# inkandswitch/peritext

Measured on NVIDIA H100. Metric: ops merged/sec across batch, higher is better.
Workload: dtype u32

## Files before the change

### peritext_b200/csrc/engine.cu

```cuda
#include <algorithm>
#include <atomic>
#include <cstdlib>
#include <cstring>
#include <initializer_list>
#include <string>
#include <thread>
#include <utility>
#include <vector>

#include "merge_kernel.cuh"
#include "warp_kernel.cuh"
#include "patch_kernel.cuh"
#include "patch_large_kernel.cuh"
#include "team_kernel.cuh"
#include "render_kernel.cuh"
#include "patch_json_kernel.cuh"
#include "append_kernel.cuh"
#include "change_kernel.cuh"
#include "exchange_kernel.cuh"
#include "changes_json_kernel.cuh"
#include "upload_kernel.cuh"
#include "scan_kernel.cuh"
#include "admit_kernel.cuh"
#include "query_kernel.cuh"
// ... 60 lines not shown

struct pt_batch {
    int device = 0;
    cudaStream_t stream = nullptr;
    int num_sms = 0;
    pt_limits limits{};
    bool have_batch = false, merged = false;
    bool patch_pool_changed = false;
    bool patch_window_changed = false;
    uint32_t n_logs = 0;
    uint64_t n_insdel = 0, n_mark = 0;
    std::vector<pt_log_desc> h_desc;
    ptp::Plan plan;
    DevBuf d_runs, d_tokens, d_run_off, d_tok_off, d_cins, d_cmarks;
    DevBuf d_desc, d_insdel, d_marks, d_order, d_counters, d_results, d_text_off, d_span_off, d_text, d_spans, d_pool, d_slab, d_retry, d_seq;
    DevBuf d_bsum, d_ctoff, d_csoff, d_ctext, d_cspans;
    DevBuf d_cdesc, d_changes, d_deps, d_admit;
    std::vector<pt_change_desc> h_cdesc;
    uint64_t n_changes = 0, n_deps = 0;
    DevBuf d_patch_recs, d_patch_items, d_patch_status;
    DevBuf d_patch_first;
    DevBuf d_large_cand, d_large_scratch;
    HostBuf h_patch_recs, h_patch_items, h_patch_status, h_patch_misc, h_patch_first;
    DevBuf d_jval, d_jvoff, d_jlink, d_jloff, d_jcom, d_jcoff;
    JsonBufs spans_json, patches_json;
    JsonBufs changes_json;
    HostBuf h_cj_status;
    DevBuf d_picnt, d_piseg, d_pibsum, d_pitmp, d_pisorted;
    uint64_t patch_cap = 0;
    bool have_changes = false;
    uint32_t adm_maxR = 1;
    const pt_insdel_rec* dp_insdel = nullptr;
    const pt_mark_rec* dp_marks = nullptr;
    HostBuf h_stage, h_results, h_text, h_spans, h_pool, h_misc, h_seq, h_ctoff, h_csoff;
    HostBuf h_chg_status, h_chg_desc, h_chg_insdel, h_chg_marks;
    HostBuf h_xch_totals, h_xch_status, h_xch_off, h_xch_delivered, h_xch_desc;
    bool have_actors = false;
    DevBuf d_anames, d_aoff, d_afirst;
    std::vector<uint64_t> h_afirst, h_abyte;
    std::vector<char> h_adense;
    HostBuf h_act_data, h_act_off, h_act_first;
    HostBuf h_syn_totals, h_syn_status, h_syn_off, h_syn_aoff, h_syn_amap;
    HostBuf h_add_totals, h_add_rank, h_add_aoff, h_add_amap;
    cudaEvent_t ev0 = nullptr, ev1 = nullptr;
    cudaStream_t side = nullptr, launch_stream = nullptr;
    cudaEvent_t ev_fork = nullptr, ev_join = nullptr;
    uint64_t launches = 0;
    cudaGraphExec_t graph_exec = nullptr;
    bool graph_ok = false, graph_tried = false;
    uint32_t merges_since_upload = 0;
    bool dl_begun = false;
    uint32_t kernels_per_merge = 0;
    uint64_t pool_used_host = 0;
};

namespace {

DevCounters* counters(const pt_batch* b) { return (DevCounters*)b->d_counters.p; }

void drop_graph(pt_batch* b) {
    if (b->graph_exec) cudaGraphExecDestroy(b->graph_exec);
    b->graph_exec = nullptr; b->graph_ok = false; b->graph_tried = false; b->merges_since_upload = 0;
}

cudaError_t launched(pt_batch* b) {
    const cudaError_t e = cudaGetLastError();
// ... 168 lines not shown
        }
    }
    switch (k) {
        case 1: return launch_bin_t<kCtaBins[1].block>(b, k, P, retry);
        case 2: return launch_bin_t<kCtaBins[2].block>(b, k, P, retry);
        case 3: return launch_bin_t<kCtaBins[3].block>(b, k, P, retry);
        default: return launch_bin_t<kCtaBins[4].block>(b, k, P, retry);
    }
}

int install_plan(pt_batch* b, const pt_packed_ops& ops, ptp::Plan&& plan, bool own_records) {
    b->n_logs = ops.n_logs; b->n_insdel = ops.n_insdel_total; b->n_mark = ops.n_mark_total;
    b->h_desc.assign(ops.logs, ops.logs + ops.n_logs);
    b->plan = std::move(plan);
    int rc;
    if ((rc = alloc_and_upload_plan(b))) return rc;
    if (own_records) {
        if ((rc = reserve_n<pt_insdel_rec>(b->d_insdel, b->n_insdel))) return rc;
        if ((rc = reserve_n<pt_mark_rec>(b->d_marks, b->n_mark))) return rc;
    }
    return PT_OK;
}

int begin_upload(pt_batch* b, const pt_packed_ops& ops, bool own_records) {
    PT_CUDA(cudaSetDevice(b->device));
    PT_CUDA(cudaStreamSynchronize(b->stream));
    b->have_batch = false; b->merged = false; b->dl_begun = false; b->have_changes = false; b->have_actors = false;
    drop_graph(b);
    ptp::Plan plan;
    if (const char* err = ptp::make_plan(ops, b->limits, b->num_sms, plan)) { g_last_error = err; return PT_ERR_INVALID; }
    return install_plan(b, ops, std::move(plan), own_records);
}

int finish_upload(pt_batch* b, const void* insdel, const void* marks, std::initializer_list<std::pair<const void*, uint64_t>> sources) {
    bool pageable = false;
    for (const auto& s : sources) {
        if (!s.second) continue;
        cudaPointerAttributes a;
        if (cudaPointerGetAttributes(&a, s.first) != cudaSuccess) { cudaGetLastError(); pageable = true; }
        else if (a.type != cudaMemoryTypeHost) pageable = true;
    }
    if (pageable) PT_CUDA(cudaStreamSynchronize(b->stream));
    b->dp_insdel = (const pt_insdel_rec*)insdel; b->dp_marks = (const pt_mark_rec*)marks;
    b->have_batch = true;
    return PT_OK;
}

template <class Q, class A, class Launch>
int run_queries(pt_batch* b, const char* fn, const char* verb, const Q* queries, uint32_t n, A* out, Launch launch) {
    if (!b || (n && (!queries || !out))) return PT_ERR_INVALID;
    if (!b->merged) { g_last_error = std::string(verb) + " before merge"; return PT_ERR_STATE; }
    if (!(b->limits.flags & PT_FLAG_EMIT_SEQUENCE)) { g_last_error = "the handle was created without PT_FLAG_EMIT_SEQUENCE"; return PT_ERR_STATE; }
    if (!n) return PT_OK;
    PT_CUDA(cudaSetDevice(b->device));
    DevBuf dq, da;
    int rc;
    if ((rc = dq.reserve((size_t)n * sizeof(Q))) || (rc = da.reserve((size_t)n * sizeof(A)))) return rc;
    cudaError_t e = cudaMemcpyAsync(dq.p, queries, (size_t)n * sizeof(Q), cudaMemcpyHostToDevice, b->stream);
    if (e == cudaSuccess) {
        launch(warp_grid(b, n, 128), 128u, (const Q*)dq.p, (A*)da.p);
        e = launched(b);
    }
    if (e == cudaSuccess) e = cudaMemcpyAsync(out, da.p, (size_t)n * sizeof(A), cudaMemcpyDeviceToHost, b->stream);
    if (e == cudaSuccess) e = cudaStreamSynchronize(b->stream);
    if (e != cudaSuccess) { g_last_error = std::string(fn) + ": " + cudaGetErrorString(e); return PT_ERR_CUDA; }
    return PT_OK;
}

int load_json_pools(pt_batch* b, const pt_json_pools* pools, const char* fn, ptr::JsonPools* P) {
    struct Pool { const uint8_t* data; const uint64_t* off; uint64_t count; DevBuf* dd; DevBuf* doff; const char* name; };
    const Pool ps[3] = {{pools->values, pools->values_off, pools->n_values, &b->d_jval, &b->d_jvoff, "values"},
                        {pools->links, pools->links_off, pools->n_links, &b->d_jlink, &b->d_jloff, "links"},
                        {pools->comments, pools->comments_off, pools->n_comments, &b->d_jcom, &b->d_jcoff, "comments"}};
    for (const Pool& p : ps) {
        if (p.count && (!p.data || !p.off)) { g_last_error = std::string(fn) + ": null " + p.name + " pool with a nonzero count"; return PT_ERR_INVALID; }
        for (uint64_t k = 0; k < p.count; k++)
// ... 402 lines not shown
        n_ch = n ? ncd[n - 1].change_off + ncd[n - 1].n_changes : 0; n_dp = n ? ncd[n - 1].dep_off + ncd[n - 1].n_deps : 0;
        if ((rc = upload_n(b, dcdesc, dch->logs, n)) || (rc = upload_n(b, ncdesc, ncd.data(), n)) ||
            (rc = reserve_n<pt_change_rec>(nch, n_ch)) || (rc = reserve_n<pt_dep_rec>(ndp, n_dp))) return rc;
        const pt_change_rec* d_dchg = dch->changes;
        const pt_dep_rec* d_ddep = dch->deps;
        if (!table_on_device) {
            if ((rc = upload_n(b, dchg, dch->changes, dch->n_changes_total)) || (rc = upload_n(b, ddep, dch->deps, dch->n_deps_total))) return rc;
            d_dchg = (const pt_change_rec*)dchg.p; d_ddep = (const pt_dep_rec*)ddep.p;
        }
        if (n) {
            pta::splice_changes_kernel<<<warp_grid(b, n, threads), threads, 0, b->stream>>>(
                (const pt_change_desc*)b->d_cdesc.p, (const pt_change_desc*)ncdesc.p, (const pt_change_desc*)dcdesc.p, n, DR,
                (const pt_change_rec*)b->d_changes.p, (const pt_dep_rec*)b->d_deps.p, d_dchg, d_ddep, (pt_change_rec*)nch.p, (pt_dep_rec*)ndp.p);
            PT_CUDA(launched(b));
        }
    }
    uint32_t bad = 0;
    PT_CUDA(cudaMemcpyAsync(&bad, abad.p, 4, cudaMemcpyDeviceToHost, b->stream));
    PT_CUDA(cudaStreamSynchronize(b->stream));
    if (bad) { g_last_error = std::string(fn) + "a resident comment rank is outside comment_map"; return PT_ERR_INVALID; }
    bool keep_actors = !(R.actor_off && R.actor_off[n] > R.actor_off[0]) && !(R.ctr_off && R.ctr_off[n] > R.ctr_off[0]);
    for (uint32_t i = 0; keep_actors && i < n; i++) keep_actors = nd[i].n_actors == b->h_desc[i].n_actors;
    b->have_actors = b->have_actors && keep_actors;
    b->have_batch = false; b->merged = false; b->dl_begun = false;
    drop_graph(b);
    b->d_insdel.swap(nins); b->d_marks.swap(nmarks);
    if (dch) {
        b->d_cdesc.swap(ncdesc); b->d_changes.swap(nch); b->d_deps.swap(ndp);
        b->h_cdesc = std::move(ncd); b->n_changes = n_ch; b->n_deps = n_dp; b->adm_maxR = maxR;
    }
    if ((rc = install_plan(b, ops, std::move(plan), true))) return rc;
    PT_CUDA(cudaStreamSynchronize(b->stream));
    b->dp_insdel = (const pt_insdel_rec*)b->d_insdel.p; b->dp_marks = (const pt_mark_rec*)b->d_marks.p;
    b->have_batch = true;
    return PT_OK;
}

int pt_batch_append(pt_batch* b, const pt_packed_ops* delta, const pt_append_remap* remap, const pt_change_table* dch) {
    if (!b || !delta || (delta->n_logs && !delta->logs)) return PT_ERR_INVALID;
    if (!b->have_batch) { g_last_error = "pt_batch_append before pt_batch_upload"; return PT_ERR_STATE; }
    return splice_append(b, "pt_batch_append: ", delta, false, remap ? *remap : pt_append_remap{}, dch, false);
}

static std::string check_change(const pt_batch* b, const pt_change_input& in, std::vector<pt_log_desc>& dd, std::vector<uint32_t>& new_elems,
                                std::vector<uint32_t>& work) {
    const uint32_t n = b->n_logs;
    if (in.n_logs != n) return "the input has " + std::to_string(in.n_logs) + " logs and the batch " + std::to_string(n);
    if (!n) return std::string();
    if (!in.actor || !in.input_off) return "null actor or input_off";
    if (in.input_off[0] != 0) return "input_off[0] is not 0";
    if ((in.input_off[n] && !in.ops) || (in.n_tokens && !in.tokens)) return "null ops or tokens with a nonzero count";
    dd.resize(n); new_elems.assign(n, 0);
    uint64_t io = 0, mo = 0;
    for (uint32_t i = 0; i < n; i++) {
        const pt_log_desc& L = b->h_desc[i];
        const uint64_t lo = in.input_off[i], hi = in.input_off[i + 1];
        if (hi < lo) return "input_off decreases at log " + std::to_string(i);
        dd[i] = pt_log_desc{io, mo, 0, 0, L.n_actors, L.max_ctr};
        const uint32_t A = in.actor[i];
        if (A == PT_CHANGE_NO_ACTOR) {
            if (hi > lo) return at(i) + "InputOperations without an actor";
            continue;
        }
        if (A >= L.n_actors) return at(i) + "actor rank " + std::to_string(A) + " >= the log's " + std::to_string(L.n_actors) + " actors";
        uint64_t next = (uint64_t)L.max_ctr + 1, last = L.max_ctr, nid = 0, nmk = 0, nel = 0;
        for (uint64_t k = lo; k < hi; k++) {
// ... 544 lines not shown
    if (count) {
        pty::AddParams A{};
        A.n_logs = n; A.T = pty::Tables{(const uint8_t*)b->d_anames.p, (const unsigned long long*)b->d_aoff.p, (const unsigned long long*)b->d_afirst.p};
        A.data = (const uint8_t*)ddata.p; A.off = (const unsigned long long*)doff.p; A.first = (const unsigned long long*)dfirst.p;
        A.fresh = (uint32_t*)dfresh.p; A.new_id = (unsigned long long*)dnew.p; A.totals = (pty::SyncTotals*)dtot.p;
        pty::add_select_kernel<<<warp_grid(b, n, 128), 128, 0, b->stream>>>(A);
        PT_CUDA(launched(b));
        PT_CUDA(cudaMemcpyAsync(tot, dtot.p, (size_t)n * sizeof(pty::SyncTotals), cudaMemcpyDeviceToHost, b->stream));
        PT_CUDA(cudaStreamSynchronize(b->stream));
        for (uint32_t i = 0; i < n; i++) if (tot[i].n_new) grow[i] = i;
    } else {
        for (uint32_t i = 0; i < n; i++) tot[i] = pty::SyncTotals{};
    }
    if ((rc = grow_tables(b, fn, grow, tot, n, (const uint8_t*)ddata.p, (const unsigned long long*)doff.p, (const unsigned long long*)dfirst.p,
                          (const unsigned long long*)dnew.p, b->h_add_aoff, b->h_add_amap, &spliced))) return rc;
    if (count) {
        const pty::Tables T{(const uint8_t*)b->d_anames.p, (const unsigned long long*)b->d_aoff.p, (const unsigned long long*)b->d_afirst.p};
        pty::add_ranks_kernel<<<warp_grid(b, n, 128), 128, 0, b->stream>>>(n, T, (const uint8_t*)ddata.p, (const unsigned long long*)doff.p,
                                                                           (const unsigned long long*)dfirst.p, (uint16_t*)drank.p);
        PT_CUDA(launched(b));
        PT_CUDA(cudaMemcpyAsync(b->h_add_rank.p, drank.p, count * 2, cudaMemcpyDeviceToHost, b->stream));
        PT_CUDA(cudaStreamSynchronize(b->stream));
    }
    *out = pt_actor_view{n, count, (const uint16_t*)b->h_add_rank.p, (const uint64_t*)b->h_add_aoff.p, (const uint16_t*)b->h_add_amap.p, spliced ? 1u : 0u};
    return PT_OK;
}

static int enqueue_merge(pt_batch* b) {
    DevCounters* c = counters(b);
    PT_CUDA(cudaMemsetAsync(c, 0, sizeof(DevCounters), b->stream));
    ptk::BatchParams P{};
    P.desc = (const pt_log_desc*)b->d_desc.p;
    P.insdel = b->dp_insdel; P.marks = b->dp_marks;
    P.results = (pt_log_result*)b->d_results.p;
    P.text_off = (const uint64_t*)b->d_text_off.p; P.span_off = (const uint64_t*)b->d_span_off.p;
    P.text = (uint32_t*)b->d_text.p; P.spans = (pt_span*)b->d_spans.p;
    P.comment_pool = (uint32_t*)b->d_pool.p; P.comment_used = &c->comment_used; P.comment_cap = b->plan.pool_cap;
    P.slab = (char*)b->d_slab.p;
    P.slab_counter = c->slab; P.slab_slots = b->plan.slab_slots;
    P.seq = (b->limits.flags & PT_FLAG_EMIT_SEQUENCE) ? (uint32_t*)b->d_seq.p : nullptr;
    P.stats = c->stats;
    P.admit = nullptr;
    if (b->have_changes && b->n_logs) {
        const auto [wpb, smem] = actor_shape(b->adm_maxR);
        if (smem > 48 * 1024) PT_CUDA(cudaFuncSetAttribute(ptadm::admit_kernel, cudaFuncAttributeMaxDynamicSharedMemorySize, (int)smem));
        ptadm::admit_kernel<<<warp_grid(b, b->n_logs, wpb * 32), wpb * 32, smem, b->stream>>>(
            (const pt_change_desc*)b->d_cdesc.p, (const pt_change_rec*)b->d_changes.p, (const pt_dep_rec*)b->d_deps.p, (const pt_log_desc*)b->d_desc.p,
            b->n_logs, b->adm_maxR, (uint32_t*)b->d_admit.p, (pt_log_result*)b->d_results.p);
        PT_CUDA(launched(b));
        P.admit = (const uint32_t*)b->d_admit.p;
    }
    { const char* e = getenv("PT_PREFETCH"); P.prefetch_next = e ? (uint32_t)atoi(e) : 0u; }
    { const char* e = getenv("PT_WARP_FLAGS"); P.warp_flags = e ? (uint32_t)atoi(e) : 0x704u; }
    { const char* e = getenv("PT_TMA"); P.use_tma = e ? (uint32_t)atoi(e) : 1u; }
    int rc;
    const uint32_t* bin_first = b->plan.bin_first;
    const bool have0 = bin_first[1] > bin_first[0], haveBlocks = bin_first[kNumBins] > bin_first[1];
    const bool fork = have0 && haveBlocks && b->side != nullptr;
    if (fork) {
        PT_CUDA(cudaEventRecord(b->ev_fork, b->stream));
        PT_CUDA(cudaStreamWaitEvent(b->side, b->ev_fork, 0));
        b->launch_stream = b->side;
        for (int k = 1; k < kNumBins; k++) if ((rc = launch_bin(b, k, P, false))) { b->launch_stream = b->stream; return rc; }
        PT_CUDA(cudaEventRecord(b->ev_join, b->side));
        b->launch_stream = b->stream;
        if ((rc = launch_bin(b, 0, P, false))) return rc;
// ... 578 lines not shown
```

### peritext_b200/csrc/merge_kernel.cuh

```cuda
#pragma once
#include <cuda_runtime.h>
#include <stdint.h>

#include "../../include/peritext_b200.h"
#include "../../include/pt_digest.h"

namespace ptk {

struct BatchParams {
    const pt_log_desc* __restrict__ desc;
    const pt_insdel_rec* __restrict__ insdel;
    const pt_mark_rec* __restrict__ marks;
    const uint32_t* __restrict__ order;
    uint32_t n_work;
    uint32_t* work_counter;
    pt_log_result* results;
    const uint64_t* __restrict__ text_off;
    const uint64_t* __restrict__ span_off;
    uint32_t* text;
    pt_span* spans;
    uint32_t* comment_pool;
    unsigned long long* comment_used;
    unsigned long long comment_cap;
    char* slab;
    unsigned long long slab_bytes;
    uint32_t* slab_counter;
    uint32_t slab_slots;
    uint32_t smem_arena_bytes;
    unsigned long long* stats;
    uint32_t* retry_list;
    uint32_t* retry_count;
    const uint32_t* n_work_dev;
    uint32_t prefetch_next;
    uint32_t warp_flags;
    uint32_t use_tma;
    uint32_t* seq;
    const uint32_t* admit;
};

__device__ __forceinline__ uint4 ld_rec(const pt_insdel_rec* p) { return __ldg(reinterpret_cast<const uint4*>(p)); }
__device__ __forceinline__ void prefetch_l2(const void* p) { asm volatile("prefetch.global.L2 [%0];" ::"l"(p)); }

__device__ __forceinline__ uint32_t smem_u32(const void* p) { return (uint32_t)__cvta_generic_to_shared(p); }
__device__ __forceinline__ void mbar_init(unsigned long long* bar, uint32_t count) {
    asm volatile("mbarrier.init.shared::cta.b64 [%0], %1;" ::"r"(smem_u32(bar)), "r"(count) : "memory");
// ... 965 lines not shown
```

### peritext_b200/csrc/plan.cpp

```cpp
#include "plan.h"

#include <algorithm>
#include <cstdio>
#include <cstdlib>
#include <numeric>

namespace ptp {

RouteConfig RouteConfig::from_env() {
    RouteConfig c;
    if (const char* f = getenv("PT_WARP_FORCE")) c.force = atoi(f) != 0;
    if (const char* t = getenv("PT_TEAM")) c.team_on = atoi(t) != 0;
    if (const char* pw = getenv("PT_PATCH_WARP")) c.patch_warp_on = atoi(pw) != 0;
    if (const char* w = getenv("PT_WARP")) {
        unsigned long a, wp, sl, ct;
        if (sscanf(w, "%lu:%lu:%lu:%lu", &a, &wp, &sl, &ct) == 4) {
            if (sl < 256) sl *= 1024;
            sl &= ~(unsigned long)15;
            if ((wp == 2 || wp == 4 || wp == 8) && sl * wp <= 227 * 1024) c.warp = BinCfg{(uint32_t)a, (int)wp * 32, (uint32_t)sl, (int)ct};
        } else if (atoi(w) == 0) {
            c.warp_on = false; c.team_on = false;
        }
    }
    return c;
}

Route route_of(const pt_log_desc& L, const RouteConfig& cfg, bool emit_sequence) {
    const uint64_t n = L.n_insdel, m = L.n_mark, R = L.n_actors ? L.n_actors : 1, recs = n + m, KS = (uint64_t)L.max_ctr * R;
    const bool key16 = !emit_sequence && KS < 0xFFFFull;
    if (cfg.warp_on && key16 && recs <= cfg.warp.max_recs) {
        const bool packed3 = R == 3 && n <= 1022, compact = R >= 3 && R <= 30 && n <= 2046;
        const uint64_t idbytes = packed3 ? 4ull * L.max_ctr : compact ? 2ull * L.max_ctr + 512 : 2 * KS;
        const uint64_t rest = packed3 ? n / 2 + 32 + 14 * (n / 4) + (KS / 32 + 2) * 6 + 512 : n / 2 + 16 * n / 3 + 1024;
        if (cfg.force || idbytes + rest <= cfg.warp.smem) return packed3 ? kPacked3 : compact ? kCompact : kDirect;
    }
    if (cfg.team_on && key16 && m == 0 && n < 0xFFFFu && (3 * n) / 4 + 2 * KS + 2 * n + 1024 <= kTeamSmem) return kTeam;
    int bin = 1;
    while (bin < kNumBins - 1 && recs > kCtaBins[bin].max_recs) bin++;
    const uint64_t I = (n < 32000 && m < 32000) ? 2 : 4, seg = std::min<uint64_t>(2 * m + 2, n / 2 + 2);
    const uint64_t typical = KS * I + (14 * n) / 10 + std::max<uint64_t>(5 * n, m ? m * (6 * I + 13) + 18 * seg : 0) + 2048;
    while (bin < kNumBins - 1 && typical > kCtaBins[bin].smem) bin++;
    return Route(kCta1 + bin - 1);
}

static size_t al16(size_t b) { return (b + 15) & ~(size_t)15; }

size_t arena_worst_bytes(uint64_t n, uint64_t m, uint64_t KS) {
    const size_t I = (n < 32000 && m < 32000) ? 2 : 4;
    size_t b = 0;
    auto A = [&](uint64_t count, size_t sz) { b += al16((size_t)count * sz); };
    const uint64_t NWr = (n + 31) / 32 + 1;
    A(KS, I); A(NWr, 4); A(NWr, 4); A(NWr, 4); A(NWr, I); A(NWr, I);
    A(NWr * 32 + 32, 1); A(NWr * 32 + 32, 1);
    A(2 * n + 3, 8); A((2 * n + 9) / 8 + 3, 8); A((2 * n + 9) / 8 + 3, 8);
    A(n + 1, I); A(n + 2, 4); A(n + 2, 4); A(n + 1, I); A(n + 1, 4); A(n + 2, I);
    A(n + 1, I); A(n + 1, I); A(n + 1, I);
    A(n / 33 + 2, I); A(KS / 32 + 2, 4); A(KS / 32 + 2, I);
    if (m) {
        const uint64_t KW = KS / 32 + 2, S = 2 * m + 2, Mc = m, nsp = 2 * m + 1, NWp = (n + 32) / 32 + 1;
        A(KW + 1, 4); A(KW + 1, I); for (int k = 0; k < 6; k++) A(m + 1, I);
        A(m + 1, 1); A(m + 1, 4); A(m + 1, 4);
        A(NWp + 1, 4); A(NWp + 1, I);
        A(2 * S + 2, 4); A(S + 1, 4); A(S + 1, 4); A(S + 2, 4);
// ... 58 lines not shown
```

### peritext_b200/csrc/upload_kernel.cuh

```cuda
#pragma once
#include <cstdint>

#include "../../include/peritext_b200.h"

namespace ptu {

__global__ void expand_runs_kernel(const pt_log_desc* __restrict__ desc, const unsigned long long* __restrict__ run_off,
                                   const unsigned long long* __restrict__ tok_off, const pt_run_rec* __restrict__ runs,
                                   const uint32_t* __restrict__ tokens, pt_insdel_rec* __restrict__ out, uint32_t n_logs) {
    const uint32_t warp = (blockIdx.x * blockDim.x + threadIdx.x) >> 5, lane = threadIdx.x & 31, nwarps = (gridDim.x * blockDim.x) >> 5;
    for (uint32_t li = warp; li < n_logs; li += nwarps) {
        const unsigned long long r0 = run_off[li], r1 = run_off[li + 1];
        pt_insdel_rec* o = out + desc[li].insdel_off;
        const uint32_t* tk = tokens + tok_off[li];
        uint32_t rec_base = 0, tok_base = 0;
        for (unsigned long long rb = r0; rb < r1; rb += 32) {
            const unsigned long long ri = rb + lane;
            uint4 r = make_uint4(0, 0, 0, 0);
            uint32_t cnt = 0, kind = 0;
            if (ri < r1) { r = __ldg(reinterpret_cast<const uint4*>(runs + ri)); cnt = r.w & 0x3FFFFFFFu; kind = r.w >> 30; }
            uint32_t tcnt = kind == PT_KIND_INSERT ? cnt : 0u;
            uint32_t pr = cnt, pt = tcnt;
#pragma unroll
            for (int d = 1; d < 32; d <<= 1) { uint32_t a = __shfl_up_sync(0xffffffffu, pr, d), b2 = __shfl_up_sync(0xffffffffu, pt, d); if (lane >= (uint32_t)d) { pr += a; pt += b2; } }
// ... 11 lines not shown
                    w.y = r.y + k; w.z = r.z; w.w = kind << 30;
                }
                reinterpret_cast<uint4*>(o)[ro + k] = w;
            }
            rec_base += tot_r; tok_base += tot_t;
        }
    }
}

__global__ void expand_insdel_c8_kernel(const pt_insdel_c8* __restrict__ in, pt_insdel_rec* __restrict__ out, unsigned long long n) {
    for (unsigned long long i = (unsigned long long)blockIdx.x * blockDim.x + threadIdx.x; i < n; i += (unsigned long long)gridDim.x * blockDim.x) {
        const uint2 q = __ldg(reinterpret_cast<const uint2*>(in + i));
        const uint32_t tok22 = q.y >> 10;
        uint4 o;
        o.x = q.x & 0xFFFFu; o.y = q.x >> 16;
        o.z = (q.y & 0xFu) | (((q.y >> 4) & 0xFu) << 16);
        o.w = (((q.y >> 8) & 3u) << 30) | ((tok22 & 0x200000u) ? PT_TOKEN_POOLED : 0u) | (tok22 & 0x1FFFFFu);
        reinterpret_cast<uint4*>(out)[i] = o;
    }
}
__global__ void expand_mark_c16_kernel(const pt_mark_c16* __restrict__ in, pt_mark_rec* __restrict__ out, unsigned long long n) {
    for (unsigned long long i = (unsigned long long)blockIdx.x * blockDim.x + threadIdx.x; i < n; i += (unsigned long long)gridDim.x * blockDim.x) {
        const uint4 q = __ldg(reinterpret_cast<const uint4*>(in + i));
        uint4 a, b;
        a.x = q.x & 0xFFFFu;
        a.y = (q.w & 0xFu) | (((q.w >> 12) & 7u) << 16) | (((q.w >> 15) & 0xFu) << 24);
        a.z = q.x >> 16; a.w = q.y & 0xFFFFu;
        b.x = ((q.w >> 4) & 0xFu) | (((q.w >> 8) & 0xFu) << 16);
        b.y = q.z; b.z = q.y >> 16; b.w = 0;
        reinterpret_cast<uint4*>(out)[2 * i] = a; reinterpret_cast<uint4*>(out)[2 * i + 1] = b;
    }
}

}
```

### peritext_b200/csrc/warp_kernel.cuh

```cuda
#pragma once
#include "merge_kernel.cuh"

namespace ptk {

constexpr uint32_t kFull = 0xffffffffu;
constexpr uint32_t kNone16 = 0xFFFFu;
constexpr uint32_t kWarpGrab = 4;
constexpr uint32_t kMaxSegSurvivorWork = 1536;
constexpr uint32_t kMaxCommentSurvivors = 48;

__device__ __forceinline__ uint32_t warp_incl_scan(uint32_t v, uint32_t lane) {
#pragma unroll
    for (int o = 1; o < 32; o <<= 1) { const uint32_t y = __shfl_up_sync(kFull, v, o); if (lane >= (uint32_t)o) v += y; }
    return v;
}

struct WArena {
    uint32_t base, used, cap;
    template <class T> __device__ __forceinline__ T* alloc(uint32_t count) {
        const uint32_t off = used;
        used += (uint32_t)((count * sizeof(T) + 15u) & ~15u);
        return reinterpret_cast<T*>(ptk_smem + base + off);
    }
    __device__ __forceinline__ bool fits() const { return used <= cap; }
// ... 28 lines not shown
#pragma unroll 1
    for (uint32_t i = lane; i < nvec; i += 32) d[i] = q;
}

#ifdef PT_PHASE_CLOCKS
enum : int { kPhStart, kPhAB, kPhC, kPhD, kPhE, kPhF, kPhG, kPhI, kPhRound, kNumPhases };
__device__ unsigned long long ptk_phase_clk[kNumPhases + 1];
struct PhaseClock {
    long long t;
    unsigned long long c[kNumPhases], logs;
    __device__ __forceinline__ void mark(int k) { const long long now = clock64(); c[k] += (unsigned long long)(now - t); t = now; }
};
#define PT_PHASE(k) pclk.mark(k)
#define PT_PHASE_PARAM , PhaseClock& pclk
#define PT_PHASE_ARG , pclk
#else
#define PT_PHASE(k) ((void)0)
#define PT_PHASE_PARAM
#define PT_PHASE_ARG
#endif

constexpr int kIdDirect = 0, kIdCompact = 1, kIdPacked3 = 2;

template <int IDM>
__device__ __forceinline__ int warp_merge_one_log(const BatchParams& P, const uint32_t li, const uint32_t slice_base, const uint32_t slice_bytes, const uint32_t li_next, PhaseSync ps PT_PHASE_PARAM) {
    const uint32_t lane = threadIdx.x & 31u;
    const uint32_t lt = (1u << lane) - 1u;

    const uint4 dsc0 = __ldg(reinterpret_cast<const uint4*>(P.desc + li)), dsc1 = __ldg(reinterpret_cast<const uint4*>(P.desc + li) + 1);
    const unsigned long long insdel_off = (unsigned long long)dsc0.x | ((unsigned long long)dsc0.y << 32);
    const unsigned long long mark_off = (unsigned long long)dsc0.z | ((unsigned long long)dsc0.w << 32);
    const uint32_t n = dsc1.x, m = dsc1.y, R = dsc1.z ? dsc1.z : 1u, C = dsc1.w;
    const unsigned long long KS64 = (unsigned long long)C * R;
    if (KS64 >= 0xFFFFull || n >= 0xFFFFu || m >= 0xFFFFu) { ps.leave(); return 1; }
    const uint32_t KS = (uint32_t)KS64;
    const pt_insdel_rec* __restrict__ ins = P.insdel + insdel_off;
    const pt_mark_rec* __restrict__ mk = P.marks + mark_off;
    uint32_t* text_out = P.text + P.text_off[li];
    pt_span* span_out = P.spans + P.span_off[li];
    pt_log_result* res = P.results + li;

    if ((P.warp_flags & 1u) && m) {
        const char* p0 = reinterpret_cast<const char*>(mk);
        const uint32_t lines = (m * (uint32_t)sizeof(pt_mark_rec) + 127u) >> 7;
        for (uint32_t l = lane; l < lines; l += 32) prefetch_l2(p0 + ((size_t)l << 7));
    }

    WArena A; A.base = slice_base; A.used = 0; A.cap = slice_bytes;
    uint32_t st = 0;
    auto keyOf = [&](uint32_t ctr, uint32_t actor) -> uint32_t { return (ctr - 1u) * R + actor; };
    auto badId = [&](uint32_t ctr, uint32_t actor) -> bool { return ctr - 1u >= C || actor >= R; };
    auto fail = [&](uint32_t code) { st |= 1u << code; };
    auto failDup = [&]() { st |= 1u; };
    auto bail = [&](uint32_t code) { if (lane == 0) { pt_log_result r{}; r.status = code; *res = r; } };

    constexpr bool compact = IDM == kIdCompact, packed = IDM == kIdPacked3;
    if (compact && !(R >= 3u && R <= 30u && n <= 2046u)) { ps.leave(); return 1; }
    if (packed && !(R == 3u && n <= 1022u)) { ps.leave(); return 1; }
    constexpr uint32_t kOvSlots = 128, kOvMax = 96, kOvEmpty = 0xFFFFFFFFu;
    const uint32_t NWr = (n + 31) / 32 + 1;
    uint32_t* OV = A.alloc<uint32_t>(compact ? kOvSlots : 0u);
    uint4* WI = A.alloc<uint4>(NWr);
    uint16_t* T = A.alloc<uint16_t>(packed ? 2u * C : compact ? C : KS);
    uint32_t* T32 = reinterpret_cast<uint32_t*>(T);
    if (!A.fits()) { ps.leave(); return 1; }
    if (packed) wfill<uint32_t>(T32, C, 0u, lane);
    else wfill<uint16_t>(T, compact ? C : KS, (uint16_t)kNone16, lane);
    if (compact) wfill<uint32_t>(OV, kOvSlots, kOvEmpty, lane);
    wfill<uint32_t>(reinterpret_cast<uint32_t*>(WI), 4 * NWr, 0u, lane);
    __syncwarp();
    auto ovHash = [&](uint32_t key) -> uint32_t { return ((key * 40503u) >> 7) & (kOvSlots - 1u); };
    auto lookup = [&](uint32_t ctr, uint32_t actor) -> uint32_t {
        if (packed) { const uint32_t f = (T32[ctr - 1u] >> (10u * actor)) & 1023u; return f ? f - 1u : kNone16; }
        if (!compact) return T[keyOf(ctr, actor)];
        const uint32_t e = T[ctr - 1u];
        if (e == kNone16) return kNone16;
        if ((e >> 11) == actor) return e & 0x7FFu;
        const uint32_t key = keyOf(ctr, actor);
        for (uint32_t h = ovHash(key);; h = (h + 1u) & (kOvSlots - 1u)) {
            const uint32_t v = OV[h];
            if (v == kOvEmpty) return kNone16;
            if ((v >> 16) == key) return v & 0xFFFFu;
        }
    };

    uint32_t nOv = 0;
    {
        uint32_t carryK = 0xFFFFFFFFu;
        const uint32_t nm1 = n ? n - 1u : 0u;
        uint4 ra = make_uint4(0, 0, 0, 0);
        if (n) ra = ld_rec(ins + min(lane, nm1));
        const char* insb = reinterpret_cast<const char*>(ins);
        const uint32_t insBytes = n * 16u;
        if (lane * 128u + 1024u < insBytes) prefetch_l2(insb + 1024u + lane * 128u);
        PT_PHASE(kPhStart);
#pragma unroll 2
        for (uint32_t base = 0; base < n; base += 32) {
            const uint32_t i = base + lane;
            if ((base & 255u) == 0u) {
                const uint32_t po = (base + 320u) * 16u + lane * 128u;
                if (po < insBytes) prefetch_l2(insb + po);
            }
            const uint4 rc = ld_rec(ins + min(i + 32u, nm1));
            const uint4 r = ra;
            const uint32_t ctr = r.x, ref_ctr = r.y, actor = r.z & 0xFFFFu, ref_actor = r.z >> 16, kind = r.w >> 30;
            const bool inb = i < n;
            const bool kbad = kind > 1u, ibad = badId(ctr, actor);
            const bool valid = inb && !kbad && !ibad;
            if (inb && kbad) fail(PT_LOG_BAD_KIND);
            if (inb && ibad) fail(PT_LOG_BAD_OPID);
            const uint32_t key = keyOf(ctr, actor);
            const bool isIns = valid && kind == PT_KIND_INSERT;
            bool toOv = false, wrote = false;
            uint32_t mine = 0;
            if (isIns) {
                if (packed) {
                    const uint32_t sh = 10u * actor;
                    if ((atomicOr(&T32[ctr - 1u], (i + 1u) << sh) >> sh) & 1023u) failDup();
                } else if (!compact) {
                    if (T[key] != kNone16) failDup();
                    T[key] = (uint16_t)i;
                } else {
                    mine = (actor << 11) | i;
                    const uint32_t e = T[ctr - 1u];
                    if (e == kNone16) { T[ctr - 1u] = (uint16_t)mine; wrote = true; }
                    else if ((e >> 11) == actor) failDup();
                    else toOv = true;
                }
            }
            const uint32_t myK = isIns ? key : 0xFFFFFFFFu;
            uint32_t prevK = __shfl_up_sync(kFull, myK, 1);
            if (lane == 0) prevK = carryK;
            carryK = __shfl_sync(kFull, myK, 31);
            const bool refOk = ref_ctr != 0 && !badId(ref_ctr, ref_actor);
            const uint32_t rkey = keyOf(ref_ctr, ref_actor);
            bool cand = isIns && refOk && rkey == prevK;
            if (cand && rkey >= key) { fail(PT_LOG_CYCLE); cand = false; }
            const uint32_t insW = __ballot_sync(kFull, isIns), candW = __ballot_sync(kFull, cand);
// ... 27 lines not shown
                const bool found = j != kNone16 && j < i;
                const bool cyc = isIns && rkey >= key;
                if (need) {
                    if (hasRef ? !found : !isIns) fail(PT_LOG_ELEM_NOT_FOUND);
                    else if (hasRef && cyc) fail(PT_LOG_CYCLE);
                }
                if (need && found && !cyc) atomicOr(reinterpret_cast<uint32_t*>(&WI[j >> 5]) + (isIns ? 2u : 3u), 1u << (j & 31));
            }
            ra = rc;
        }
    }
    __syncwarp();
    ps.pass();
    if (compact && nOv > kOvMax) { ps.leave(); return 1; }
    st = __reduce_or_sync(kFull, st);
    if (st) { bail(st > 1u ? 31u - __clz(st) : PT_LOG_BAD_OPID); ps.leave(); return 0; }
    PT_PHASE(kPhAB);

    uint32_t M, nvis, N = 0;
    {
        uint32_t carryH = 0, carryV = 0, otherCarry = 0;
        for (uint32_t wb = 0; wb < NWr; wb += 32) {
            const uint32_t w = wb + lane;
            uint32_t insW = 0, candW = 0, otherW = 0, delW = 0;
            if (w < NWr) { const uint4 q = WI[w]; insW = q.x; candW = q.y; otherW = q.z; delW = q.w; }
            const uint32_t up = __shfl_up_sync(kFull, otherW, 1);
            const uint32_t prevBit = lane ? (up >> 31) : otherCarry;
            otherCarry = __shfl_sync(kFull, otherW, 31) >> 31;
            const uint32_t head = insW & (~candW | ((otherW << 1) | prevBit));
            const uint32_t vis = insW & ~delW;
            const uint32_t pc = __popc(head) | (__popc(vis) << 16);
            const uint32_t inc = warp_incl_scan(pc, lane), ex = inc - pc, tot = __shfl_sync(kFull, inc, 31);
            if (w < NWr) WI[w] = make_uint4(insW, head, vis, (carryH + (ex & 0xFFFFu)) | ((carryV + (ex >> 16)) << 16));
#pragma unroll
            for (uint32_t k = 0; k < 4; k++)
                if ((head >> (8u * k)) & 0xFFu) prefetch_l2(ins + w * 32u + 8u * k);
            carryH += tot & 0xFFFFu; carryV += tot >> 16;
            N += __reduce_add_sync(kFull, (uint32_t)__popc(insW));
        }
        M = carryH; nvis = carryV;
    }
    __syncwarp();
    PT_PHASE(kPhC);

    auto runOf = [&](uint32_t i) -> uint32_t {
        const uint4 q = WI[i >> 5];
        return (q.w & 0xFFFFu) + __popc(q.y & (0xFFFFFFFFu >> (31 - (i & 31)))) - 1u;
    };
    auto visBefore = [&](uint32_t i) -> uint32_t {
        const uint4 q = WI[i >> 5];
        return (q.w >> 16) + __popc(q.z & ((1u << (i & 31)) - 1u));
    };

    if ((P.warp_flags & 2u) && li_next != 0xFFFFFFFFu && lane == 0) prefetch_l2(P.desc + li_next);
    const uint32_t E = 2 * (M + 1), END = (E + 7u) & ~7u;
    if (END + 1 >= 0xFFFFu) { ps.leave(); return 1; }
    uint16_t* VisBase = A.alloc<uint16_t>(M + 1);
    const uint32_t markD = A.used;
    {
        const uint32_t SPEND = END >> 3, nSp = SPEND + 2, KW = (KS + 31) / 32;
        uint32_t* Node = A.alloc<uint32_t>(E);
        uint16_t* N16 = reinterpret_cast<uint16_t*>(Node);
        uint16_t* HV = A.alloc<uint16_t>(M + 1);
        uint16_t* Prun = A.alloc<uint16_t>(M + 1);
        uint16_t* RKey = A.alloc<uint16_t>(M + 2);
        uint16_t* Last = RKey;
        auto ByG = [&](uint32_t pos) -> uint16_t& { return N16[2 * ((M + 1) + pos) + 1]; };
        const uint32_t uBytes = max((uint32_t)(((KW + 1) * 4 + 15) & ~15u) + (uint32_t)(((KW + 1) * 2 + 15) & ~15u), 2u * (uint32_t)((nSp * 4 + 15) & ~15u));
        char* U = A.alloc<char>(uBytes);
        if (!A.fits()) { ps.leave(); return 1; }
        uint32_t* KBits = reinterpret_cast<uint32_t*>(U);
        uint16_t* KPre = reinterpret_cast<uint16_t*>(U + (((KW + 1) * 4 + 15) & ~15u));
        uint32_t* Sub = reinterpret_cast<uint32_t*>(U);
        uint32_t* Sub2 = reinterpret_cast<uint32_t*>(U + ((nSp * 4 + 15) & ~15u));
#pragma unroll 1
        for (uint32_t wb = 0; wb < NWr; wb += 32) {
            const uint32_t w = wb + lane;
            if (w < NWr) {
                const uint4 q = WI[w];
                uint32_t hb = q.y, rid = q.w & 0xFFFFu;
                while (hb) { const uint32_t b = __ffs(hb) - 1; hb &= hb - 1; HV[rid++] = (uint16_t)(w * 32 + b); }
            }
        }
        wfill<uint32_t>(KBits, KW + 1, 0u, lane);
        __syncwarp();
#pragma unroll 1
        for (uint32_t rb = 0; rb < M; rb += 32) {
            const uint32_t r = rb + lane;
            if (r < M) {
                const uint32_t i = HV[r], w = i >> 5, b = i & 31;
                const uint4 rec = ld_rec(ins + i);
                const uint4 q0 = WI[w];
                uint32_t stop = (q0.y | ~q0.x) & ~(0xFFFFFFFFu >> (31 - b));
                uint32_t ww = w;
                while (!stop) { ww++; const uint2 q1 = *reinterpret_cast<const uint2*>(&WI[ww]); stop = q1.y | ~q1.x; }
                const uint32_t end = ww * 32 + (__ffs(stop) - 1);
                const uint32_t key = keyOf(rec.x, rec.z & 0xFFFFu);
                const uint32_t p = rec.y == 0 ? n : lookup(rec.y, rec.z >> 16);
                const uint32_t q = p == n ? M : runOf(p);
                const uint32_t hv = visBefore(i);
                N16[2 * r + 1] = (uint16_t)(visBefore(end) - hv);
                HV[r] = (uint16_t)hv;
                Prun[r] = (uint16_t)q; RKey[r] = (uint16_t)key;
                atomicOr(&KBits[key >> 5], 1u << (key & 31));
            }
        }
        __syncwarp();
        {
            uint32_t carry = 0;
#pragma unroll 1
            for (uint32_t wb = 0; wb < KW; wb += 32) {
                const uint32_t w = wb + lane;
                const uint32_t cnt = w < KW ? __popc(KBits[w]) : 0u;
                const uint32_t inc = warp_incl_scan(cnt, lane);
                if (w < KW) KPre[w] = (uint16_t)(carry + inc - cnt);
                carry += __shfl_sync(kFull, inc, 31);
            }
        }
        __syncwarp();
#pragma unroll 1
        for (uint32_t rb = 0; rb < M; rb += 32) {
            const uint32_t r = rb + lane;
            if (r < M) {
                const uint32_t key = RKey[r];
                ByG((uint32_t)KPre[key >> 5] + __popc(KBits[key >> 5] & ((1u << (key & 31)) - 1u))) = (uint16_t)r;
            }
        }
        __syncwarp();
        ps.pass();
        wfill<uint16_t>(Last, M + 2, (uint16_t)kNone16, lane);
        __syncwarp();
// ... 61 lines not shown
            Sub = cur;
        }
#pragma unroll 1
        for (uint32_t rb = 0; rb < M; rb += 32) {
            const uint32_t r = rb + lane;
            if (r < M) {
                const uint32_t a = Node[r];
                const uint32_t suf = (Sub[a & 0xFFFFu] >> 16) - (a >> 16);
                VisBase[r] = (uint16_t)((nvis - suf) - (uint32_t)HV[r]);
            }
        }
        __syncwarp();
    }
    A.used = markD;
    ps.pass();
    PT_PHASE(kPhE);

    uint16_t* EV = A.alloc<uint16_t>(n + 1);
    if (!A.fits() || nvis >= 0x8000u) { ps.leave(); return 1; }
    unsigned long long d0 = 0, d1 = 0;
#pragma unroll 1
    for (uint32_t w = 0; w + 1 < NWr; w++) {
        const uint4 q = WI[w];
        const uint32_t ib = q.x;
        if (!ib) continue;
        const uint32_t hbits = q.y, vbits = q.z, hp = q.w & 0xFFFFu, vp = q.w >> 16;
        if ((ib >> lane) & 1u) {
            const uint32_t i = w * 32 + lane;
            const uint32_t run = hp + __popc(hbits & (0xFFFFFFFFu >> (31 - lane))) - 1u;
            const uint32_t vr = ((uint32_t)VisBase[run] + vp + __popc(vbits & lt)) & 0xFFFFu;
            const uint32_t isv = (vbits >> lane) & 1u;
            EV[i] = (uint16_t)(vr | (isv << 15));
            if (isv) {
                const uint32_t tok = PT_PAYLOAD_TOKEN(__ldg(&ins[i].payload));
                text_out[vr] = tok;
                digest_add(d0, d1, pt_term_text(vr, tok));
            }
        }
    }
    __syncwarp();

    uint32_t nspans = 0;
    if ((P.warp_flags & 2u) && li_next != 0xFFFFFFFFu) {
        const uint4 q0 = __ldg(reinterpret_cast<const uint4*>(P.desc + li_next)), q1 = __ldg(reinterpret_cast<const uint4*>(P.desc + li_next) + 1);
        const char* p0 = reinterpret_cast<const char*>(P.insdel + ((unsigned long long)q0.x | ((unsigned long long)q0.y << 32)));
        const uint32_t lines = (q1.x * (uint32_t)sizeof(pt_insdel_rec) + 127u) >> 7;
        for (uint32_t l = lane; l < lines; l += 32) prefetch_l2(p0 + ((size_t)l << 7));
    }

    if (m) {
        const uint32_t pfb = min(m * 32u, 6u * 1024u);
        for (uint32_t o = lane * 128u; o < pfb; o += 32u * 128u) prefetch_l2(reinterpret_cast<const char*>(mk) + o);
    }
    PT_PHASE(kPhF);
    uint32_t nS = 0, nC = 0;
    uint4* Sv = nullptr;
    uint16_t* CIdx = nullptr;
    if (m) {
        const uint32_t KW = (KS + 31) / 32;
        uint32_t* KBits = A.alloc<uint32_t>(KW + 1);
        CIdx = A.alloc<uint16_t>(kMaxCommentSurvivors + 32);
        if (!A.fits()) { ps.leave(); return 1; }
        const uint32_t room = A.cap - A.used, svStart = A.used;
        uint32_t capS = room > 256u ? (room - 256u) / 16u : 0u;
        if (capS > m) capS = m;
        Sv = A.alloc<uint4>(capS + 1);
        if (!A.fits()) { ps.leave(); return 1; }
        wfill<uint32_t>(KBits, KW + 1, 0u, lane);
        __syncwarp();
        const uint4* mq = reinterpret_cast<const uint4*>(mk);
        const uint32_t mm1 = m - 1u;
        uint4 a0 = __ldg(mq + 2 * min(lane, mm1)), a1 = __ldg(mq + 2 * min(lane, mm1) + 1);
        const uint32_t mkBytes = m * 32u;
#pragma unroll 2
        for (uint32_t kb = 0; kb < m; kb += 32) {
            const uint32_t k = kb + lane;
            if ((kb & 127u) == 0u) {
                const uint32_t po = (kb + 192u) * 32u + lane * 128u;
                if (po < mkBytes) prefetch_l2(reinterpret_cast<const char*>(mk) + po);
            }
            const uint32_t kn = min(k + 32u, mm1);
            const uint4 b0 = __ldg(mq + 2 * kn), b1 = __ldg(mq + 2 * kn + 1);
            const uint32_t ctr = a0.x, actor = a0.y & 0xFFFFu, kind = (a0.y >> 16) & 0xFFu, bounds = a0.y >> 24;
            const uint32_t start_ctr = a0.z, end_ctr = a0.w, start_actor = a1.x & 0xFFFFu, end_actor = a1.x >> 16, attr = a1.y, arrival = a1.z;
            const uint32_t type = (kind >> 1) & 3u;
            const bool inb = k < m;
            const bool idok = inb && !badId(ctr, actor);
            const uint32_t key = keyOf(ctr, actor);
            bool dup = false;
            if (idok) {
                const uint32_t bit = 1u << (key & 31);
                dup = (atomicOr(&KBits[key >> 5], bit) & bit) != 0 || lookup(ctr, actor) != kNone16;
            }
            if (inb && (!idok || dup)) fail(PT_LOG_BAD_OPID);
            const uint32_t sb = bounds & 3u, eb = (bounds >> 2) & 3u;
            const bool sOk = idok && sb <= PT_BOUND_AFTER && !badId(start_ctr, start_actor);
            uint32_t js = kNone16;
            if (sOk) js = lookup(start_ctr, start_actor);
            const bool sHit = js != kNone16 && js < arrival;
            uint32_t es = 0;
            if (sHit) es = EV[js];
            const uint32_t va = (es & 0x7FFFu) + (sb & (es >> 15));
            const bool eOk = sHit && eb <= PT_BOUND_AFTER && !badId(end_ctr, end_actor);
            uint32_t je = kNone16;
            if (eOk) je = lookup(end_ctr, end_actor);
            const bool eHit = je != kNone16 && je < arrival && !(je == js && eb == sb);
            uint32_t vb = nvis;
            if (eHit) { const uint32_t ee = EV[je]; vb = (ee & 0x7FFFu) + (eb & (ee >> 15)); }
            const bool surv = sHit && va < vb;
            const bool isC = surv && type == PT_MARK_COMMENT;
            const uint32_t bal = __ballot_sync(kFull, surv), balC = __ballot_sync(kFull, isC);
            if (surv) {
                const uint32_t idx = nS + __popc(bal & lt);
                if (idx < capS) {
                    Sv[idx] = make_uint4(va | (vb << 16), (type == PT_MARK_COMMENT ? k : key) | (kind << 16), attr, 0u);
                    if (isC) { const uint32_t ci = nC + __popc(balC & lt); if (ci <= kMaxCommentSurvivors) CIdx[ci] = (uint16_t)idx; }
                }
            }
            nS += __popc(bal); nC += __popc(balC);
            a0 = b0; a1 = b1;
        }
        __syncwarp();
        st = __reduce_or_sync(kFull, st);
        if (st) { bail(31u - __clz(st)); ps.leave(); return 0; }
        if (nS > capS) { ps.leave(); return 1; }
        A.used = svStart + ((nS * 16u + 15u) & ~15u);
    }

    ps.pass();
    PT_PHASE(kPhG);
    unsigned long long pool_base = 0;
    if (nvis == 0) nspans = 0;
    else if (nS == 0) {
        if (lane == 0) {
            pt_span s; s.start = 0; s.flags = 0; s.link_attr = PT_ATTR_NONE; s.comment_off = 0;
            span_out[0] = s;
            digest_add(d0, d1, pt_term_span(0, 0, 0, PT_ATTR_NONE));
        }
        nspans = 1;
    } else {
        if (nC > kMaxCommentSurvivors) { ps.leave(); return 1; }
        if (nvis <= 32u && nC <= 32u) {
            const uint32_t x = lane;
            uint32_t w0 = 0, w1 = 0, w2 = 0, flags = 0, link = PT_ATTR_NONE;
#pragma unroll 1
            for (uint32_t j = 0; j < nS; j++) {
                const uint4 sv = Sv[j];
                const uint32_t ab = sv.x, pk = sv.y;
                const bool cover = x >= (ab & 0xFFFFu) && x < (ab >> 16);
                const uint32_t t = (pk >> 17) & 3u, val = (((pk & 0xFFFFu) << 16) | j) + 1u;
                if (cover) {
                    if (t == PT_MARK_STRONG) w0 = max(w0, val);
                    else if (t == PT_MARK_EM) w1 = max(w1, val);
// ... 320 lines not shown
```

Before: 89.10 billion.

## Derive compact half-width insdel and mark records for the warp merge path

At upload and append time, a new kernel packs each 16-byte insdel record into 8 bytes and each 32-byte mark record into 16 bytes. Counters become 16-bit and actors 8-bit, using saturating casts. The warp merge kernel then reads these compact arrays, with prefetch distances and line counts rescaled, and still reads the full record for the text payload. This halves the record bytes the warp route loads. In exchange it adds a conversion pass and extra device memory, and it routes logs with more than 255 actors off the warp path. Mark kind is kept to 3 bits, which assumes kind values stay small.

```diff
diff --git a/peritext_b200/csrc/engine.cu b/peritext_b200/csrc/engine.cu
--- a/peritext_b200/csrc/engine.cu
+++ b/peritext_b200/csrc/engine.cu
@@ -116,6 +116,7 @@
     uint32_t adm_maxR = 1;
     const pt_insdel_rec* dp_insdel = nullptr;
     const pt_mark_rec* dp_marks = nullptr;
+    DevBuf d_half_insdel, d_half_marks;
     HostBuf h_stage, h_results, h_text, h_spans, h_pool, h_misc, h_seq, h_ctoff, h_csoff;
     HostBuf h_chg_status, h_chg_desc, h_chg_insdel, h_chg_marks;
     HostBuf h_xch_totals, h_xch_status, h_xch_off, h_xch_delivered, h_xch_desc;
@@ -350,6 +351,21 @@
     return install_plan(b, ops, std::move(plan), own_records);
 }
 
+int derive_half_records(pt_batch* b) {
+    const uint32_t* nr = b->plan.n_route;
+    if (!(nr[ptp::kPacked3] + nr[ptp::kCompact] + nr[ptp::kDirect])) { b->d_half_insdel.release(); b->d_half_marks.release(); return PT_OK; }
+    int rc;
+    if ((rc = reserve_n<uint2>(b->d_half_insdel, b->n_insdel)) || (rc = reserve_n<uint4>(b->d_half_marks, b->n_mark))) return rc;
+    const uint64_t total = b->n_insdel + b->n_mark;
+    const uint32_t threads = 256;
+    if (total) {
+        ptu::derive_half_records_kernel<<<warp_grid(b, total, threads, 1), threads, 0, b->stream>>>(
+            b->dp_insdel, b->dp_marks, (uint2*)b->d_half_insdel.p, (uint4*)b->d_half_marks.p, b->n_insdel, b->n_mark);
+        PT_CUDA(launched(b));
+    }
+    return PT_OK;
+}
+
 int finish_upload(pt_batch* b, const void* insdel, const void* marks, std::initializer_list<std::pair<const void*, uint64_t>> sources) {
     bool pageable = false;
     for (const auto& s : sources) {
@@ -358,8 +374,10 @@
         if (cudaPointerGetAttributes(&a, s.first) != cudaSuccess) { cudaGetLastError(); pageable = true; }
         else if (a.type != cudaMemoryTypeHost) pageable = true;
     }
+    b->dp_insdel = (const pt_insdel_rec*)insdel; b->dp_marks = (const pt_mark_rec*)marks;
+    int rc;
+    if ((rc = derive_half_records(b))) return rc;
     if (pageable) PT_CUDA(cudaStreamSynchronize(b->stream));
-    b->dp_insdel = (const pt_insdel_rec*)insdel; b->dp_marks = (const pt_mark_rec*)marks;
     b->have_batch = true;
     return PT_OK;
 }
@@ -828,6 +846,7 @@
     if ((rc = install_plan(b, ops, std::move(plan), true))) return rc;
     PT_CUDA(cudaStreamSynchronize(b->stream));
     b->dp_insdel = (const pt_insdel_rec*)b->d_insdel.p; b->dp_marks = (const pt_mark_rec*)b->d_marks.p;
+    if ((rc = derive_half_records(b))) return rc;
     b->have_batch = true;
     return PT_OK;
 }
@@ -1438,6 +1457,7 @@
     ptk::BatchParams P{};
     P.desc = (const pt_log_desc*)b->d_desc.p;
     P.insdel = b->dp_insdel; P.marks = b->dp_marks;
+    P.half_insdel = (const uint2*)b->d_half_insdel.p; P.half_marks = (const uint4*)b->d_half_marks.p;
     P.results = (pt_log_result*)b->d_results.p;
     P.text_off = (const uint64_t*)b->d_text_off.p; P.span_off = (const uint64_t*)b->d_span_off.p;
     P.text = (uint32_t*)b->d_text.p; P.spans = (pt_span*)b->d_spans.p;
diff --git a/peritext_b200/csrc/merge_kernel.cuh b/peritext_b200/csrc/merge_kernel.cuh
--- a/peritext_b200/csrc/merge_kernel.cuh
+++ b/peritext_b200/csrc/merge_kernel.cuh
@@ -11,6 +11,8 @@
     const pt_log_desc* __restrict__ desc;
     const pt_insdel_rec* __restrict__ insdel;
     const pt_mark_rec* __restrict__ marks;
+    const uint2* __restrict__ half_insdel;
+    const uint4* __restrict__ half_marks;
     const uint32_t* __restrict__ order;
     uint32_t n_work;
     uint32_t* work_counter;
diff --git a/peritext_b200/csrc/plan.cpp b/peritext_b200/csrc/plan.cpp
--- a/peritext_b200/csrc/plan.cpp
+++ b/peritext_b200/csrc/plan.cpp
@@ -28,7 +28,7 @@
 Route route_of(const pt_log_desc& L, const RouteConfig& cfg, bool emit_sequence) {
     const uint64_t n = L.n_insdel, m = L.n_mark, R = L.n_actors ? L.n_actors : 1, recs = n + m, KS = (uint64_t)L.max_ctr * R;
     const bool key16 = !emit_sequence && KS < 0xFFFFull;
-    if (cfg.warp_on && key16 && recs <= cfg.warp.max_recs) {
+    if (cfg.warp_on && key16 && R <= 255 && recs <= cfg.warp.max_recs) {
         const bool packed3 = R == 3 && n <= 1022, compact = R >= 3 && R <= 30 && n <= 2046;
         const uint64_t idbytes = packed3 ? 4ull * L.max_ctr : compact ? 2ull * L.max_ctr + 512 : 2 * KS;
         const uint64_t rest = packed3 ? n / 2 + 32 + 14 * (n / 4) + (KS / 32 + 2) * 6 + 512 : n / 2 + 16 * n / 3 + 1024;
diff --git a/peritext_b200/csrc/upload_kernel.cuh b/peritext_b200/csrc/upload_kernel.cuh
--- a/peritext_b200/csrc/upload_kernel.cuh
+++ b/peritext_b200/csrc/upload_kernel.cuh
@@ -67,4 +67,22 @@
     }
 }
 
+__device__ __forceinline__ uint32_t sat16(uint32_t v) { return min(v, 0xFFFFu); }
+__device__ __forceinline__ uint32_t sat8(uint32_t v) { return min(v, 0xFFu); }
+__global__ void derive_half_records_kernel(const pt_insdel_rec* __restrict__ ins, const pt_mark_rec* __restrict__ mk,
+                                           uint2* __restrict__ hins, uint4* __restrict__ hmk, unsigned long long n, unsigned long long m) {
+    for (unsigned long long i = (unsigned long long)blockIdx.x * blockDim.x + threadIdx.x; i < n + m; i += (unsigned long long)gridDim.x * blockDim.x) {
+        if (i < n) {
+            const uint4 r = __ldg(reinterpret_cast<const uint4*>(ins + i));
+            hins[i] = make_uint2(sat16(r.x) | (sat16(r.y) << 16), sat8(r.z & 0xFFFFu) | (sat8(r.z >> 16) << 8) | ((r.w >> 30) << 16));
+        } else {
+            const uint4* q = reinterpret_cast<const uint4*>(mk + (i - n));
+            const uint4 a = __ldg(q), b = __ldg(q + 1);
+            hmk[i - n] = make_uint4(sat16(a.x) | (sat16(a.z) << 16), sat16(a.w) | (sat16(b.z) << 16), b.y,
+                                    sat8(a.y & 0xFFFFu) | (sat8(b.x & 0xFFFFu) << 8) | (sat8(b.x >> 16) << 16) |
+                                        (((a.y >> 16) & 7u) << 24) | (((a.y >> 24) & 0xFu) << 27));
+        }
+    }
 }
+
+}
diff --git a/peritext_b200/csrc/warp_kernel.cuh b/peritext_b200/csrc/warp_kernel.cuh
--- a/peritext_b200/csrc/warp_kernel.cuh
+++ b/peritext_b200/csrc/warp_kernel.cuh
@@ -84,17 +84,18 @@
     const unsigned long long mark_off = (unsigned long long)dsc0.z | ((unsigned long long)dsc0.w << 32);
     const uint32_t n = dsc1.x, m = dsc1.y, R = dsc1.z ? dsc1.z : 1u, C = dsc1.w;
     const unsigned long long KS64 = (unsigned long long)C * R;
-    if (KS64 >= 0xFFFFull || n >= 0xFFFFu || m >= 0xFFFFu) { ps.leave(); return 1; }
+    if (KS64 >= 0xFFFFull || n >= 0xFFFFu || m >= 0xFFFFu || R > 255u) { ps.leave(); return 1; }
     const uint32_t KS = (uint32_t)KS64;
-    const pt_insdel_rec* __restrict__ ins = P.insdel + insdel_off;
-    const pt_mark_rec* __restrict__ mk = P.marks + mark_off;
+    const uint2* __restrict__ ins = P.half_insdel + insdel_off;
+    const uint4* __restrict__ mk = P.half_marks + mark_off;
+    const pt_insdel_rec* __restrict__ full_ins = P.insdel + insdel_off;
     uint32_t* text_out = P.text + P.text_off[li];
     pt_span* span_out = P.spans + P.span_off[li];
     pt_log_result* res = P.results + li;
 
     if ((P.warp_flags & 1u) && m) {
         const char* p0 = reinterpret_cast<const char*>(mk);
-        const uint32_t lines = (m * (uint32_t)sizeof(pt_mark_rec) + 127u) >> 7;
+        const uint32_t lines = (m * 16u + 127u) >> 7;
         for (uint32_t l = lane; l < lines; l += 32) prefetch_l2(p0 + ((size_t)l << 7));
     }
 
@@ -140,22 +141,22 @@
     {
         uint32_t carryK = 0xFFFFFFFFu;
         const uint32_t nm1 = n ? n - 1u : 0u;
-        uint4 ra = make_uint4(0, 0, 0, 0);
-        if (n) ra = ld_rec(ins + min(lane, nm1));
+        uint2 ra = make_uint2(0, 0);
+        if (n) ra = __ldg(ins + min(lane, nm1));
         const char* insb = reinterpret_cast<const char*>(ins);
-        const uint32_t insBytes = n * 16u;
-        if (lane * 128u + 1024u < insBytes) prefetch_l2(insb + 1024u + lane * 128u);
+        const uint32_t insBytes = n * 8u;
+        if (lane * 128u + 512u < insBytes) prefetch_l2(insb + 512u + lane * 128u);
         PT_PHASE(kPhStart);
 #pragma unroll 2
         for (uint32_t base = 0; base < n; base += 32) {
             const uint32_t i = base + lane;
-            if ((base & 255u) == 0u) {
-                const uint32_t po = (base + 320u) * 16u + lane * 128u;
+            if ((base & 511u) == 0u) {
+                const uint32_t po = (base + 576u) * 8u + lane * 128u;
                 if (po < insBytes) prefetch_l2(insb + po);
             }
-            const uint4 rc = ld_rec(ins + min(i + 32u, nm1));
-            const uint4 r = ra;
-            const uint32_t ctr = r.x, ref_ctr = r.y, actor = r.z & 0xFFFFu, ref_actor = r.z >> 16, kind = r.w >> 30;
+            const uint2 rc = __ldg(ins + min(i + 32u, nm1));
+            const uint2 r = ra;
+            const uint32_t ctr = r.x & 0xFFFFu, ref_ctr = r.x >> 16, actor = r.y & 0xFFu, ref_actor = (r.y >> 8) & 0xFFu, kind = r.y >> 16;
             const bool inb = i < n;
             const bool kbad = kind > 1u, ibad = badId(ctr, actor);
             const bool valid = inb && !kbad && !ibad;
@@ -249,9 +250,8 @@
             const uint32_t pc = __popc(head) | (__popc(vis) << 16);
             const uint32_t inc = warp_incl_scan(pc, lane), ex = inc - pc, tot = __shfl_sync(kFull, inc, 31);
             if (w < NWr) WI[w] = make_uint4(insW, head, vis, (carryH + (ex & 0xFFFFu)) | ((carryV + (ex >> 16)) << 16));
-#pragma unroll
-            for (uint32_t k = 0; k < 4; k++)
-                if ((head >> (8u * k)) & 0xFFu) prefetch_l2(ins + w * 32u + 8u * k);
+            if (head & 0xFFFFu) prefetch_l2(ins + w * 32u);
+            if (head >> 16) prefetch_l2(ins + w * 32u + 16u);
             carryH += tot & 0xFFFFu; carryV += tot >> 16;
             N += __reduce_add_sync(kFull, (uint32_t)__popc(insW));
         }
@@ -306,14 +306,14 @@
             const uint32_t r = rb + lane;
             if (r < M) {
                 const uint32_t i = HV[r], w = i >> 5, b = i & 31;
-                const uint4 rec = ld_rec(ins + i);
+                const uint2 rec = __ldg(ins + i);
                 const uint4 q0 = WI[w];
                 uint32_t stop = (q0.y | ~q0.x) & ~(0xFFFFFFFFu >> (31 - b));
                 uint32_t ww = w;
                 while (!stop) { ww++; const uint2 q1 = *reinterpret_cast<const uint2*>(&WI[ww]); stop = q1.y | ~q1.x; }
                 const uint32_t end = ww * 32 + (__ffs(stop) - 1);
-                const uint32_t key = keyOf(rec.x, rec.z & 0xFFFFu);
-                const uint32_t p = rec.y == 0 ? n : lookup(rec.y, rec.z >> 16);
+                const uint32_t key = keyOf(rec.x & 0xFFFFu, rec.y & 0xFFu), ref_ctr = rec.x >> 16;
+                const uint32_t p = ref_ctr == 0 ? n : lookup(ref_ctr, (rec.y >> 8) & 0xFFu);
                 const uint32_t q = p == n ? M : runOf(p);
                 const uint32_t hv = visBefore(i);
                 N16[2 * r + 1] = (uint16_t)(visBefore(end) - hv);
@@ -441,7 +441,7 @@
             const uint32_t isv = (vbits >> lane) & 1u;
             EV[i] = (uint16_t)(vr | (isv << 15));
             if (isv) {
-                const uint32_t tok = PT_PAYLOAD_TOKEN(__ldg(&ins[i].payload));
+                const uint32_t tok = PT_PAYLOAD_TOKEN(__ldg(&full_ins[i].payload));
                 text_out[vr] = tok;
                 digest_add(d0, d1, pt_term_text(vr, tok));
             }
@@ -452,13 +452,13 @@
     uint32_t nspans = 0;
     if ((P.warp_flags & 2u) && li_next != 0xFFFFFFFFu) {
         const uint4 q0 = __ldg(reinterpret_cast<const uint4*>(P.desc + li_next)), q1 = __ldg(reinterpret_cast<const uint4*>(P.desc + li_next) + 1);
-        const char* p0 = reinterpret_cast<const char*>(P.insdel + ((unsigned long long)q0.x | ((unsigned long long)q0.y << 32)));
-        const uint32_t lines = (q1.x * (uint32_t)sizeof(pt_insdel_rec) + 127u) >> 7;
+        const char* p0 = reinterpret_cast<const char*>(P.half_insdel + ((unsigned long long)q0.x | ((unsigned long long)q0.y << 32)));
+        const uint32_t lines = (q1.x * 8u + 127u) >> 7;
         for (uint32_t l = lane; l < lines; l += 32) prefetch_l2(p0 + ((size_t)l << 7));
     }
 
     if (m) {
-        const uint32_t pfb = min(m * 32u, 6u * 1024u);
+        const uint32_t pfb = min(m * 16u, 6u * 1024u);
         for (uint32_t o = lane * 128u; o < pfb; o += 32u * 128u) prefetch_l2(reinterpret_cast<const char*>(mk) + o);
     }
     PT_PHASE(kPhF);
@@ -477,21 +477,19 @@
         if (!A.fits()) { ps.leave(); return 1; }
         wfill<uint32_t>(KBits, KW + 1, 0u, lane);
         __syncwarp();
-        const uint4* mq = reinterpret_cast<const uint4*>(mk);
         const uint32_t mm1 = m - 1u;
-        uint4 a0 = __ldg(mq + 2 * min(lane, mm1)), a1 = __ldg(mq + 2 * min(lane, mm1) + 1);
-        const uint32_t mkBytes = m * 32u;
+        uint4 a = __ldg(mk + min(lane, mm1));
+        const uint32_t mkBytes = m * 16u;
 #pragma unroll 2
         for (uint32_t kb = 0; kb < m; kb += 32) {
             const uint32_t k = kb + lane;
-            if ((kb & 127u) == 0u) {
-                const uint32_t po = (kb + 192u) * 32u + lane * 128u;
+            if ((kb & 255u) == 0u) {
+                const uint32_t po = (kb + 384u) * 16u + lane * 128u;
                 if (po < mkBytes) prefetch_l2(reinterpret_cast<const char*>(mk) + po);
             }
-            const uint32_t kn = min(k + 32u, mm1);
-            const uint4 b0 = __ldg(mq + 2 * kn), b1 = __ldg(mq + 2 * kn + 1);
-            const uint32_t ctr = a0.x, actor = a0.y & 0xFFFFu, kind = (a0.y >> 16) & 0xFFu, bounds = a0.y >> 24;
-            const uint32_t start_ctr = a0.z, end_ctr = a0.w, start_actor = a1.x & 0xFFFFu, end_actor = a1.x >> 16, attr = a1.y, arrival = a1.z;
+            const uint4 b = __ldg(mk + min(k + 32u, mm1));
+            const uint32_t ctr = a.x & 0xFFFFu, start_ctr = a.x >> 16, end_ctr = a.y & 0xFFFFu, arrival = a.y >> 16, attr = a.z;
+            const uint32_t actor = a.w & 0xFFu, start_actor = (a.w >> 8) & 0xFFu, end_actor = (a.w >> 16) & 0xFFu, kind = (a.w >> 24) & 7u, bounds = a.w >> 27;
             const uint32_t type = (kind >> 1) & 3u;
             const bool inb = k < m;
             const bool idok = inb && !badId(ctr, actor);
@@ -527,7 +525,7 @@
                 }
             }
             nS += __popc(bal); nC += __popc(balC);
-            a0 = b0; a1 = b1;
+            a = b;
         }
         __syncwarp();
         st = __reduce_or_sync(kFull, st);
```

New measurement: 97.74 billion (median of 6 runs). +9.7%, better.
